# StevenWang30/R-PCC

Hardware: AMD Instinct MI355X
Metric: frames/s (64E, 64x2048 range img), projection->segmentation->model->quantise (higher is better)
Workload: dtype f32

## Files before the change

r-pcc_amd/csrc/fps_kernels.h:

```cpp
#pragma once

#define FPS_TAB_ROWS 12
#define FPS_TILE 256
#define FPS_TROWS 8

struct FpsTiling {
    int N;
    int W, H;
    int tcols;
    int T;
};
static inline FpsTiling fps_tiling_range(int H, int W) {
    FpsTiling g;
    g.N = H * W; g.W = W; g.H = H; g.tcols = (W + 31) / 32; g.T = ((H + FPS_TROWS - 1) / FPS_TROWS) * g.tcols;
    return g;
}
static inline FpsTiling fps_tiling_list(int N) {
    FpsTiling g;
    g.N = N; g.W = 0; g.H = 0; g.tcols = 0; g.T = (N + FPS_TILE - 1) / FPS_TILE;
    return g;
}

struct FpsLds {
    float4 *lo4;
// ... 115 lines not shown
    for (int e = 0; e < 4; e++) { bx[e] = cand[e] ? x[e] : qnan; by[e] = cand[e] ? y[e] : qnan; bz[e] = cand[e] ? z[e] : qnan; }
#pragma unroll
    for (int e = 0; e < 4; e += 2) {
        lo[0] = fmin3_raw(lo[0], bx[e], bx[e + 1]); hi[0] = fmax3_raw(hi[0], bx[e], bx[e + 1]);
        lo[1] = fmin3_raw(lo[1], by[e], by[e + 1]); hi[1] = fmax3_raw(hi[1], by[e], by[e + 1]);
        lo[2] = fmin3_raw(lo[2], bz[e], bz[e + 1]); hi[2] = fmax3_raw(hi[2], bz[e], bz[e + 1]);
    }
    dpp_box6(lo[0], lo[1], lo[2], hi[0], hi[1], hi[2]);
}

template <bool RANGE>
__device__ __forceinline__ void fps_load_point(const float *__restrict__ src, const float *__restrict__ rays, int k,
                                               float &x, float &y, float &z) {
    if (RANGE) {
        const float r = ld_f32(src, (uint32_t)k * 4u);
        x = r * ld_f32(rays, (uint32_t)k * 12u); y = r * ld_f32(rays, (uint32_t)k * 12u + 4u); z = r * ld_f32(rays, (uint32_t)k * 12u + 8u);
    } else {
        x = src[3 * (int64_t)k]; y = src[3 * (int64_t)k + 1]; z = src[3 * (int64_t)k + 2];
    }
}

struct FpsTileOut { float lo[3], hi[3], wt, wx, wy, wz; uint32_t widx; };

template <bool RANGE, bool VEC, bool EDGE = false>
__device__ __forceinline__ bool fps_tile_update(const FpsQuad &q, bool org_on, float t_org0, float c0, float c1, float c2,
                                                float *__restrict__ temp, bool with_box, FpsTileOut &o, bool &viol) {
    float x[4], y[4], z[4], nt[4];
    uint32_t key[4];
    bool cand[4], ch = false;
    fps_quad_xyz(q, RANGE, x, y, z);
    const bool lane_ok = q.nval > 0;
    constexpr bool QUAD = VEC && !EDGE;
#pragma unroll
    for (int e = 0; e < 4; e++) {
        float tp = (QUAD ? lane_ok : e < q.nval) ? q.tp[e] : -1.0f;
        if (RANGE && org_on && q.r[e] == 0.0f) {
            if (with_box) viol |= (QUAD ? lane_ok : e < q.nval) && tp != t_org0;
            tp = -1.0f;
        }
        cand[e] = tp >= 0.0f;
        const float dx = x[e] - c0, dy = y[e] - c1, dz = z[e] - c2;
        const float d = (dx * dx + dy * dy) + dz * dz;
        nt[e] = d < tp ? d : tp;
        key[e] = fps_val_key(nt[e]);
        const bool c = nt[e] != tp;
        ch |= c;
        if ((!VEC || (EDGE && q.nval != 4)) && c) st_f32(temp, (uint32_t)(q.p0 + e) * 4u, nt[e]);
        if (!c) nt[e] = q.tp[e];
    }
    if (QUAD && ch) st_at(reinterpret_cast<float4 *>(temp), (uint32_t)q.p0 * 4u, make_float4(nt[0], nt[1], nt[2], nt[3]));
    if (VEC && EDGE && ch && q.nval == 4) st_quad<true>(temp, (uint32_t)q.p0 * 4u, nt[0], nt[1], nt[2], nt[3]);
    if (!with_box && __ballot(ch) == 0ull) return false;
    if (with_box) fps_tile_box(x, y, z, cand, o.lo, o.hi);
    fps_tile_argmax(x, y, z, key, q.p0, o.wt, o.wx, o.wy, o.wz, o.widx);
    return true;
}

#define FPS_THREADS 1024

#define FPS_TT_BATCH 512
#define FPS_TT_SMALL 1024
#define FPS_GROUP 2
#define FPS_FLAG_FINALIZE_TEMP 1
#define FPS_FLAG_PROBED 2

template <bool RANGE, bool VEC, int FPS_TT>
__global__ __launch_bounds__(FPS_TT) void fps_tiled_kernel(const float *__restrict__ src, const float *__restrict__ rays,
                                                           float *__restrict__ temp, const int32_t *__restrict__ info,
                                                           FpsTiling g, int M, int flags, int32_t *__restrict__ out_idx,
                                                           float *__restrict__ out_cen,
                                                           const float *__restrict__ tiletab) {
    extern __shared__ __attribute__((aligned(16))) unsigned char fps_smem[];
    __shared__ unsigned long long red[FPS_TT / 64];
    __shared__ int redt[FPS_TT / 64];
    __shared__ int wcount, s_viol;
    const int T = g.T, N = g.N;
    FpsLds L(fps_smem, T);
    const int b = blockIdx.x, tid = threadIdx.x, lane = tid & 63, wave = tid >> 6;
    src += (int64_t)b * N * (RANGE ? 1 : 3);
    temp += (int64_t)b * N;
    out_idx += (int64_t)b * M;
    if (out_cen) out_cen += (int64_t)b * M * 3;
    if (M <= 0) return;
    if (!RANGE && (flags & FPS_FLAG_PROBED) && out_idx[0] < 0) return;

    int old = 0;
    if (RANGE) { old = info[RPCC_INFO * b + 1]; if (old >= N) old = 0; }
// ... 152 lines not shown
#pragma unroll
            for (int gi = 0; gi < GROUP; gi++) {
                const int ee = e + gi * NW;
                tt[gi] = (int)L.work[ee < n ? ee : n - 1];
                locate(tt[gi], q[gi]);
                fps_quad_load<RANGE, VEC>(src, rays, temp, q[gi]);
            }
#pragma unroll
            for (int gi = 0; gi < GROUP; gi++) if (e + gi * NW < n) compute_tile(tt[gi], q[gi], false);
        }
        __syncthreads();
        if (tid == 0) wcount = 0;
        select_next();
        if (lane == 0 && wave == (j & (NW - 1))) { out_idx[j] = old; if (out_cen) { out_cen[3 * j] = c0; out_cen[3 * j + 1] = c1; out_cen[3 * j + 2] = c2; } }
    }
    if (RANGE && org_on && (flags & FPS_FLAG_FINALIZE_TEMP)) {
        for (int p = tid; p < N; p += FPS_TT) {
            const float r = ld_f32(src, (uint32_t)p * 4u), tv = ld_f32(temp, (uint32_t)p * 4u);
            if (r == 0.0f && tv >= 0.0f && tv != t_org) st_f32(temp, (uint32_t)p * 4u, t_org);
        }
    }
}

template <bool RANGE, bool VEC, int FPS_TT, bool SOA, bool EDGE = false, int TPL = 1>
__device__ __forceinline__ void fps_regtab_body(const float *__restrict__ src, const float *__restrict__ rays,
                                                float *__restrict__ temp, const int32_t *__restrict__ info,
                                                FpsTiling g, int M, int flags, int32_t *__restrict__ out_idx,
                                                float *__restrict__ out_cen, const float *__restrict__ tiletab,
                                                const float *__restrict__ rays_soa, const int b) {
    constexpr int NW = FPS_TT / 64;
    TRACE_FPS_DECLS();
    TRACE_FPS_WG(0);
    __shared__ uint2 slot_k[2][NW];
    __shared__ float4 slot_c[2][NW];
    __shared__ int s_viol;
    const int T = g.T, N = g.N;
    const int tid = threadIdx.x, lane = tid & 63, wave = tid >> 6;
    src += (int64_t)b * N * (RANGE ? 1 : 3);
    temp += (int64_t)b * N;
    out_idx += (int64_t)b * M;
    if (out_cen) out_cen += (int64_t)b * M * 3;
    if (M <= 0) return;
    if (!RANGE && (flags & FPS_FLAG_PROBED) && out_idx[0] < 0) return;

    int old = 0;
    if (RANGE) { old = info[RPCC_INFO * b + 1]; if (old >= N) old = 0; }
    float c0, c1, c2;
    fps_load_point<RANGE>(src, rays, old, c0, c1, c2);
    if (tid == 0) {
        out_idx[0] = old;
        if (out_cen) { out_cen[0] = c0; out_cen[1] = c1; out_cen[2] = c2; }
        s_viol = 0;
    }
    int org_idx = N;
    if (RANGE) { org_idx = info[RPCC_INFO * b + 4]; if (org_idx < 0 || org_idx > N) org_idx = N; }
    bool org_on = RANGE && org_idx < N;
    float t_org = -1.0f;
// ... 77 lines not shown
            TRACE_FPS_VISIT(0);
#pragma unroll
            for (int u = 0; u < FPS_VISIT; u++) {
                on[u] = m != 0ull;
                l[u] = on[u] ? (int)__ffsll((long long)m) - 1 : l[0];
                sl[u] = on[u] ? cur : sl[0];
                m &= m - 1ull;
                if (TPL > 1) next();
                if (u < FPS_VISIT_UNCOND || on[u]) {
                    locate(l[u], sl[u], q[u]);
                    fps_quad_load<RANGE, VEC, SOA, EDGE>(src, SOA ? rays_soa : rays, temp, q[u], N);
                }
            }
            TRACE_FPS_VISIT(1);
#pragma unroll
            for (int u = 0; u < FPS_VISIT; u++) {
                FpsTileOut o;
                if (on[u] && fps_tile_update<RANGE, VEC, EDGE>(q[u], org_on, t_org0, c0, c1, c2, temp, with_box, o, viol)) store_entry(l[u], sl[u], o, with_box);
            }
            TRACE_FPS_VISIT(2);
        }
        if (with_box && __ballot(viol) != 0ull && lane == 0) s_viol = 1;
    };
    auto update_origin = [&]() {
        if (org_on) {
            const float d = (c0 * c0 + c1 * c1) + c2 * c2;
            t_org = d < t_org ? d : t_org;
        }
    };
    int par = 0;
    auto select_next = [&]() {
        uint32_t key = have[0] ? fps_val_key(tmax[0]) : 0u, targ_b = targ[0];
        float cx_b = cx[0], cy_b = cy[0], cz_b = cz[0];
#pragma unroll
        for (int t = 1; t < TPL; t++) {
            const uint32_t k1 = have[t] ? fps_val_key(tmax[t]) : 0u;
            const bool sec = k1 > key || (k1 == key && targ[t] < targ_b);
            key = sec ? k1 : key; targ_b = sec ? targ[t] : targ_b;
            cx_b = sec ? cx[t] : cx_b; cy_b = sec ? cy[t] : cy_b; cz_b = sec ? cz[t] : cz_b;
        }
        uint32_t vmax = dpp_max_u32(key);
        unsigned long long mm = __ballot(key == vmax);
        uint32_t imin;
        if (__popcll(mm) == 1) {
            imin = (uint32_t)__builtin_amdgcn_readlane((int)targ_b, (int)__ffsll((long long)mm) - 1);
        } else {
            imin = dpp_min_u32(key == vmax ? targ_b : 0xFFFFFFFFu);
            mm = __ballot(key == vmax && targ_b == imin);
        }
        {
            const int wl = mm ? (int)__ffsll((long long)mm) - 1 : 0;
            const float wx = u2f((uint32_t)__builtin_amdgcn_readlane((int)f2u(cx_b), wl));
            const float wy = u2f((uint32_t)__builtin_amdgcn_readlane((int)f2u(cy_b), wl));
            const float wz = u2f((uint32_t)__builtin_amdgcn_readlane((int)f2u(cz_b), wl));
            if (lane == 0) { slot_k[par][wave] = make_uint2(vmax, vmax >= FPS_KEY_MIN ? imin : 0xFFFFFFFFu); slot_c[par][wave] = make_float4(wx, wy, wz, 0.0f); }
        }
        TRACE_FPS_PHASE(3);
        __syncthreads();
        TRACE_FPS_PHASE(4);
        const uint2 kv = slot_k[par][lane % NW];
        const float4 cc = slot_c[par][lane % NW];
        par ^= 1;
        vmax = NW == 8 ? dpp_max8_u32(kv.x) : dpp_max_u32(kv.x);
        mm = __ballot(kv.x == vmax) & ((1ull << NW) - 1ull);
        if (__popcll(mm) == 1) {
            imin = (uint32_t)__builtin_amdgcn_readlane((int)kv.y, (int)__ffsll((long long)mm) - 1);
        } else {
            imin = dpp_min_u32(kv.x == vmax ? kv.y : 0xFFFFFFFFu);
            mm = __ballot(kv.x == vmax && kv.y == imin);
        }
        const int wl = mm ? (int)__ffsll((long long)mm) - 1 : 0;
        const uint32_t okey = org_on ? fps_val_key(t_org) : 0u;
        if (okey >= FPS_KEY_MIN && (okey > vmax || (okey == vmax && (uint32_t)org_idx < imin))) {
            old = org_idx;
            fps_load_point<RANGE>(src, rays, org_idx, c0, c1, c2);
        } else if (vmax < FPS_KEY_MIN || imin == 0xFFFFFFFFu) {
            old = 0;
            fps_load_point<RANGE>(src, rays, 0, c0, c1, c2);
        } else {
            old = (int)imin;
            c0 = u2f((uint32_t)__builtin_amdgcn_readlane((int)f2u(cc.x), wl));
            c1 = u2f((uint32_t)__builtin_amdgcn_readlane((int)f2u(cc.y), wl));
            c2 = u2f((uint32_t)__builtin_amdgcn_readlane((int)f2u(cc.z), wl));
        }
    };

    const bool have_tab = RANGE && tiletab != nullptr && info[RPCC_INFO * b + 3] == 1;
    if (M > 1 && have_tab) {
#pragma unroll
        for (int s = 0; s < TPL; s++) {
            if (have[s]) {
                const float4 *t4 = reinterpret_cast<const float4 *>(tiletab + (int64_t)b * FPS_TAB_ROWS * T);
                const float4 a = t4[my_t[s]], h = t4[T + my_t[s]], c = t4[2 * T + my_t[s]];
                lo0[s] = a.x; lo1[s] = a.y; lo2[s] = a.z; tmax[s] = a.w; hi0[s] = h.x; hi1[s] = h.y; hi2[s] = h.z; targ[s] = f2u(h.w);
                cx[s] = c.x; cy[s] = c.y; cz[s] = c.z;
            }
        }
        update_origin();
    } else if (M > 1) {
        __syncthreads();
        visit(have_m, true);
        __syncthreads();
        if (org_on && s_viol) {
            org_on = false; t_org = -1.0f;
            visit(have_m, true);
        }
        update_origin();
    }
    if (M > 1) {
        select_next();
        if (tid == 0) { out_idx[1] = old; if (out_cen) { out_cen[3] = c0; out_cen[4] = c1; out_cen[5] = c2; } }
    }
    TRACE_FPS_PHASE(0);
    for (int j = 2; j < M; j++) {
        unsigned long long vm[TPL];
#pragma unroll
        for (int s = 0; s < TPL; s++) {
            const float g0 = fmaxf(fmaxf(lo0[s] - c0, c0 - hi0[s]), 0.0f);
            const float g1 = fmaxf(fmaxf(lo1[s] - c1, c1 - hi1[s]), 0.0f);
            const float g2 = fmaxf(fmaxf(lo2[s] - c2, c2 - hi2[s]), 0.0f);
            const float bound = (g0 * g0 + g1 * g1) + g2 * g2;
            vm[s] = __ballot(have[s] && bound < tmax[s]);
        }
        TRACE_FPS_TILES(vm[0], j);
        TRACE_FPS_PHASE(1);
        visit(vm, false);
        TRACE_FPS_PHASE(2);
        update_origin();
        select_next();
        if (lane == 0 && wave == (j & (NW - 1))) { out_idx[j] = old; if (out_cen) { out_cen[3 * j] = c0; out_cen[3 * j + 1] = c1; out_cen[3 * j + 2] = c2; } }
        TRACE_FPS_PHASE(5);
    }
    TRACE_FPS_WG(1);
    if (RANGE && org_on && (flags & FPS_FLAG_FINALIZE_TEMP)) {
        __syncthreads();
        for (int p = tid; p < N; p += FPS_TT) {
            const float r = ld_f32(src, (uint32_t)p * 4u), tv = ld_f32(temp, (uint32_t)p * 4u);
            if (r == 0.0f && tv >= 0.0f && tv != t_org) st_f32(temp, (uint32_t)p * 4u, t_org);
        }
    }
}

template <bool RANGE, bool VEC, int FPS_TT, bool EDGE = false>
__global__ __launch_bounds__(FPS_TT) __attribute__((amdgpu_waves_per_eu(4, 8))) void fps_regtab_kernel(
    const float *__restrict__ src, const float *__restrict__ rays, float *__restrict__ temp, const int32_t *__restrict__ info, FpsTiling g, int M,
    int flags, int32_t *__restrict__ out_idx, float *__restrict__ out_cen, const float *__restrict__ tiletab) {
    fps_regtab_body<RANGE, VEC, FPS_TT, false, EDGE>(src, rays, temp, info, g, M, flags, out_idx, out_cen, tiletab, nullptr, blockIdx.x);
}
template <int FPS_TT, bool EDGE = false>
__global__ __launch_bounds__(FPS_TT) __attribute__((amdgpu_waves_per_eu(5, 8))) void fps_regtab_planar_kernel(
    const float *__restrict__ src, const float *__restrict__ rays, float *__restrict__ temp, const int32_t *__restrict__ info, FpsTiling g, int M,
    int flags, int32_t *__restrict__ out_idx, float *__restrict__ out_cen, const float *__restrict__ tiletab, const float *__restrict__ rays_soa) {
    fps_regtab_body<true, true, FPS_TT, true, EDGE>(src, rays, temp, info, g, M, flags, out_idx, out_cen, tiletab, rays_soa, blockIdx.x);
}
template <int FPS_TT, bool EDGE = false>
__global__ __launch_bounds__(FPS_TT) __attribute__((amdgpu_waves_per_eu(4, 8))) void fps_regtab_planar2_kernel(
    const float *__restrict__ src, const float *__restrict__ rays, float *__restrict__ temp, const int32_t *__restrict__ info, FpsTiling g, int M,
    int flags, int32_t *__restrict__ out_idx, float *__restrict__ out_cen, const float *__restrict__ tiletab, const float *__restrict__ rays_soa) {
    fps_regtab_body<true, true, FPS_TT, true, EDGE, 2>(src, rays, temp, info, g, M, flags, out_idx, out_cen, tiletab, rays_soa, blockIdx.x);
}
struct FpsGroupArgs {
    const float *src, *rays;
    float *temp;
    const int32_t *info;
    FpsTiling g;
    int32_t *out_idx;
    float *out_cen;
    const float *tiletab, *rays_soa;
};
struct FpsMulti {
    int n, first[RPCC_MAX_GROUPS + 1];
    int edge[RPCC_MAX_GROUPS];
    FpsGroupArgs a[RPCC_MAX_GROUPS];
};
template <int FPS_TT>
__global__ __launch_bounds__(FPS_TT) __attribute__((amdgpu_waves_per_eu(5, 8))) void fps_regtab_planar_multi_kernel(const FpsMulti m, int M, int flags) {
    const int gi = multi_group_of(m.first, m.n, blockIdx.x);
    const FpsGroupArgs &a = m.a[gi];
    const int b = (int)blockIdx.x - m.first[gi];
    if (m.edge[gi]) fps_regtab_body<true, true, FPS_TT, true, true>(a.src, a.rays, a.temp, a.info, a.g, M, flags, a.out_idx, a.out_cen, a.tiletab, a.rays_soa, b);
    else            fps_regtab_body<true, true, FPS_TT, true, false>(a.src, a.rays, a.temp, a.info, a.g, M, flags, a.out_idx, a.out_cen, a.tiletab, a.rays_soa, b);
}

#define TAB_TPW 2
#define MASK_WAVES 4
#define MASK_VGPR_ATTR
template <bool RAW, bool VEC, bool EDGE = false>
__global__ __launch_bounds__(64 * MASK_WAVES) MASK_VGPR_ATTR void ground_mask_tab_kernel(float *__restrict__ ri, const float *__restrict__ tm,
                                                              const double *__restrict__ ground, double thr, FpsTiling g,
                                                              float *__restrict__ temp, int32_t *__restrict__ info,
                                                              float *__restrict__ tiletab) {
    __shared__ int s_cnt[MASK_WAVES], s_nz[MASK_WAVES], s_first[MASK_WAVES], s_forg[MASK_WAVES];
    const int b = blockIdx.y, lane = threadIdx.x & 63, wave = threadIdx.x >> 6;
    const int P = g.N, T = g.T;
    float *ri_b = ri + (int64_t)b * P, *temp_b = temp + (int64_t)b * P;
    float4 *tab4 = reinterpret_cast<float4 *>(tiletab + (int64_t)b * FPS_TAB_ROWS * T);
    int cnt = 0, nzc = 0, first = P, forg = P;
    const int t0 = (blockIdx.x * MASK_WAVES + wave) * TAB_TPW;
    const int lrow = lane >> 3, lcol = 4 * (lane & 7);
    const float pr = ri_b[min(lane, P - 1)];
    const f32x3 pray = ld_at(reinterpret_cast<const f32x3 *>(tm), (uint32_t)min(lane, P - 1) * 12u);
    FpsQuad q[TAB_TPW];
#pragma unroll
    for (int k = 0; k < TAB_TPW; k++) {
// ... 134 lines not shown
```

r-pcc_amd/csrc/rpcc_hip.hip:

```cpp
#include <hip/hip_runtime.h>
#include <limits.h>
#include <math.h>
#include <stdint.h>
#include <stdio.h>
#include <string.h>

#include <algorithm>
#include <mutex>
#include <new>
#include <type_traits>
#include <utility>
#include <vector>
#include "../../include/rpcc_hip.h"
#include "rpcc_device.h"

using namespace rpcc;

static thread_local char g_err[512] = "";
static int set_err(int code, const char *fmt, const char *a = "", const char *b = "") {
    snprintf(g_err, sizeof(g_err), fmt, a, b);
    return code;
}
#define HIP_TRY(expr)                                                                      \
    do {                                                                                   \
        hipError_t e_ = (expr);                                                            \
        if (e_ != hipSuccess) return set_err(RPCC_ERR_HIP, "%s: %s", #expr, hipGetErrorString(e_)); \
    } while (0)
// ... 1942 lines not shown
static FpsPick fps_pick_range(int H, int W, int frames, int flags, bool quads16, bool planar) {
    const FpsTiling g = fps_tiling_range(H, W);
    if (flags & RPCC_FPS_MODE_BITS) return {FPS_MODES, FPS_THREADS, false};
    if ((flags & RPCC_FPS_BRUTEFORCE) || !fps_prunable(g)) return {FPS_ONE_PASS, FPS_THREADS, false};
    return fps_pick_pruned(g, frames, quads16, planar);
}

template <bool RANGE, int TT, bool VEC>
static int launch_fps_family(FpsFamily family, const FpsGroupArgs &a, int B, int M, int kflags, hipStream_t st) {
    if constexpr (RANGE) {
        if (family == FPS_PLANAR) fps_regtab_planar_kernel<TT, !VEC><<<B, TT, 0, st>>>(a.src, a.rays, a.temp, a.info, a.g, M, kflags, a.out_idx, a.out_cen, a.tiletab, a.rays_soa);
        if (family == FPS_PLANAR2) fps_regtab_planar2_kernel<TT, !VEC><<<B, TT, 0, st>>>(a.src, a.rays, a.temp, a.info, a.g, M, kflags, a.out_idx, a.out_cen, a.tiletab, a.rays_soa);
    }
    if (family == FPS_REG_TABLE)
        fps_regtab_kernel<RANGE, RANGE || VEC, TT, RANGE && !VEC><<<B, TT, 0, st>>>(a.src, a.rays, a.temp, a.info, a.g, M, kflags, a.out_idx, a.out_cen, a.tiletab);
    if (family == FPS_LDS_TABLE) {
        const size_t sh = fps_tiled_lds_bytes(a.g.T);
        HIP_TRY(ensure_dyn_lds(reinterpret_cast<const void *>(&fps_tiled_kernel<RANGE, VEC, TT>), (int)sh));
        fps_tiled_kernel<RANGE, VEC, TT><<<B, TT, sh, st>>>(a.src, a.rays, a.temp, a.info, a.g, M, kflags, a.out_idx, a.out_cen, a.tiletab);
    }
    LAUNCH_CHECK();
    return RPCC_OK;
}
template <bool RANGE>
static int launch_fps_tiled(const FpsPick &k, const FpsGroupArgs &a, int B, int M, int kflags, hipStream_t st) {
    if (k.threads == FPS_TT_SMALL)
        return k.unaligned ? launch_fps_family<RANGE, FPS_TT_SMALL, false>(k.family, a, B, M, kflags, st) : launch_fps_family<RANGE, FPS_TT_SMALL, true>(k.family, a, B, M, kflags, st);
    return k.unaligned ? launch_fps_family<RANGE, FPS_TT_BATCH, false>(k.family, a, B, M, kflags, st) : launch_fps_family<RANGE, FPS_TT_BATCH, true>(k.family, a, B, M, kflags, st);
}

static int fps_xyz_impl(int B, int N, int M, const float *points, float *temp, int32_t *idx, bool brute, hipStream_t st, int flags = 0) {
    ARG_TRY(B > 0 && B <= RPCC_MAX_BATCH && N > 0 && M >= 0 && points && temp && idx);
    ARG_TRY(!((flags & RPCC_FPS_FMA1) && (flags & RPCC_FPS_FMA2)));
    if (M == 0) return RPCC_OK;
    if (flags & RPCC_FPS_MODE_BITS) {
        fps_modes_kernel<false><<<B, FPS_THREADS, 0, st>>>(points, nullptr, temp, nullptr, N, M, fps_fma_of(flags),
                                                           (flags & RPCC_FPS_TIE_CUDA) ? 1 : 0, fps_pow2_down_mask(), idx, nullptr);
        LAUNCH_CHECK();
        return RPCC_OK;
    }
    const FpsTiling g = fps_tiling_list(N);
    const bool vec = (N % 4 == 0) && aligned16(points) && aligned16(temp);
    int probed = 0;
    if (!brute && fps_prunable(g)) {
        fps_list_probe_kernel<<<B, 256, 0, st>>>(points, N, M, g.T, idx);
        LAUNCH_CHECK();
        const int rc = launch_fps_tiled<false>(fps_pick_pruned(g, B, vec, false), {points, nullptr, temp, nullptr, g, idx, nullptr, nullptr, nullptr}, B, M, FPS_FLAG_PROBED, st);
        if (rc != RPCC_OK) return rc;
// ... 1289 lines not shown
    }
    if (m.n == 0) return RPCC_OK;
    return launch_ground_ransac_multi(m, st);
}
static int mixed_fps(const BatchPlan *pl, int G, hipStream_t st) {
    int rc, total = 0, tt = FPS_TT_SMALL;
    for (int i = 0; i < G; i++)
        if (pl[i].tiled && pl[i].io->timer == nullptr) total += pl[i].Bs;
    bool common[RPCC_MAX_GROUPS];
    FpsMulti m;
    m.n = 0; m.first[0] = 0;
    for (int i = 0; i < G; i++) {
        const BatchPlan &p = pl[i];
        const FpsPick k = fps_pick_range(p.g.H, p.g.W, total, p.io->flags, range_quads16(p.g.W, p.io->ri, p.temp, p.io->tm), true);
        common[i] = k.family == FPS_PLANAR && p.io->timer == nullptr;
        if (!common[i]) continue;
        tt = k.threads;
        m.a[m.n] = {p.io->ri, p.io->tm, p.temp, p.io->info, fps_tiling_range(p.g.H, p.g.W), p.io->cen_pix, p.io->centers, p.tiletab, p.rays_soa};
        m.edge[m.n] = k.unaligned ? 1 : 0;
        m.first[m.n + 1] = m.first[m.n] + p.Bs;
        m.n++;
    }
    if (m.n > 0) {
        if (tt == FPS_TT_SMALL) fps_regtab_planar_multi_kernel<FPS_TT_SMALL><<<m.first[m.n], FPS_TT_SMALL, 0, st>>>(m, pl[0].M, 0);
        else                    fps_regtab_planar_multi_kernel<FPS_TT_BATCH><<<m.first[m.n], FPS_TT_BATCH, 0, st>>>(m, pl[0].M, 0);
        LAUNCH_CHECK();
    }
    for (int i = 0; i < G; i++)
        if (!common[i] && (rc = run_stage<uint8_t>(pl[i], ST_FPS, st))) return rc;
    return RPCC_OK;
}
static int mixed_planes(const BatchPlan *pl, int G, hipStream_t st) {
    PlaneMulti m;
    m.n = 0; m.first[0] = 0;
    const int M = pl[0].M, K = M + 2, wpg = PL_THREADS / 64, groups = (K + wpg - 1) / wpg;
    for (int i = 0; i < G; i++) {
        const BatchPlan &p = pl[i];
        if (p.io->model_method == 0) continue;
        m.a[m.n] = plane_group_args(p.io->tm, p.io->ground, p.Bs, p.P, M, p.io->plane_cos_cut, (uint32_t)p.io->plane_seed, p.io->frame_ids,
                                    p.io->model, p.io->counts, p.ws, p.extra, nullptr);
        m.first[m.n + 1] = m.first[m.n] + p.Bs * (K - 2) + p.Bs * groups;
        m.n++;
    }
    if (m.n == 0) return RPCC_OK;
    plane_model_multi_kernel<10><<<m.first[m.n], PL_THREADS, 0, st>>>(m, M, kpad(M), PL_BIG);
    LAUNCH_CHECK();
    return RPCC_OK;
}
// ... 233 lines not shown
```

Measured before the change: 358,500.

## Speculatively process two FPS centres per round with guessed next centre

Adds a speculative 'pair' mode to the tiled FPS kernel. Each round updates distances for the current centre and also for a guessed next centre, which is the runner-up candidate still valid after the current update. The second centre's tile updates are staged in LDS and committed only if the guess proves correct, so one barrier and reduction round can yield two centres. It also emits v_subrev with a scalar operand for the distance subtraction. The cost is extra LDS staging, more register pressure, pause/backoff logic when staging overflows, and correctness risk, which a new simulator script is meant to check.

```diff
diff --git a/r-pcc_amd/csrc/fps_kernels.h b/r-pcc_amd/csrc/fps_kernels.h
--- a/r-pcc_amd/csrc/fps_kernels.h
+++ b/r-pcc_amd/csrc/fps_kernels.h
@@ -161,6 +161,24 @@
 
 struct FpsTileOut { float lo[3], hi[3], wt, wx, wy, wz; uint32_t widx; };
 
+__device__ __forceinline__ float fps_point_min(float x, float y, float z, float c0, float c1, float c2, float tp) {
+    const float dx = x - c0, dy = y - c1, dz = z - c2;
+    const float d = (dx * dx + dy * dy) + dz * dz;
+    return d < tp ? d : tp;
+}
+__device__ __forceinline__ float fps_sub_uniform(float x, float c) {
+    float r;
+    asm("v_subrev_f32_e32 %0, %1, %2" : "=v"(r) : "s"(c), "v"(x));
+    return r;
+}
+template <bool UNI>
+__device__ __forceinline__ float fps_point_min_t(float x, float y, float z, float c0, float c1, float c2, float tp) {
+    if (!UNI) return fps_point_min(x, y, z, c0, c1, c2, tp);
+    const float dx = fps_sub_uniform(x, c0), dy = fps_sub_uniform(y, c1), dz = fps_sub_uniform(z, c2);
+    const float d = (dx * dx + dy * dy) + dz * dz;
+    return d < tp ? d : tp;
+}
+
 template <bool RANGE, bool VEC, bool EDGE = false>
 __device__ __forceinline__ bool fps_tile_update(const FpsQuad &q, bool org_on, float t_org0, float c0, float c1, float c2,
                                                 float *__restrict__ temp, bool with_box, FpsTileOut &o, bool &viol) {
@@ -178,9 +196,7 @@
             tp = -1.0f;
         }
         cand[e] = tp >= 0.0f;
-        const float dx = x[e] - c0, dy = y[e] - c1, dz = z[e] - c2;
-        const float d = (dx * dx + dy * dy) + dz * dz;
-        nt[e] = d < tp ? d : tp;
+        nt[e] = fps_point_min(x[e], y[e], z[e], c0, c1, c2, tp);
         key[e] = fps_val_key(nt[e]);
         const bool c = nt[e] != tp;
         ch |= c;
@@ -195,13 +211,87 @@
     return true;
 }
 
+template <bool RANGE, bool VEC, bool EDGE = false>
+__device__ __forceinline__ void fps_pair_begin(const FpsQuad &q, bool org_on, bool in_b, float4 *__restrict__ stage, float (&x)[4], float (&y)[4],
+                                               float (&z)[4], float (&tp)[4]) {
+    fps_quad_xyz(q, RANGE, x, y, z);
+    const bool lane_ok = q.nval > 0;
+    constexpr bool QUAD = VEC && !EDGE;
+    if (in_b) *stage = make_float4(q.tp[0], q.tp[1], q.tp[2], q.tp[3]);
+#pragma unroll
+    for (int e = 0; e < 4; e++) {
+        tp[e] = (QUAD ? lane_ok : e < q.nval) ? q.tp[e] : -1.0f;
+        if (RANGE && org_on && q.r[e] == 0.0f) tp[e] = -1.0f;
+    }
+}
+template <bool VEC, bool EDGE = false>
+__device__ __forceinline__ bool fps_pair_centre(const FpsQuad &q, const float (&x)[4], const float (&y)[4], const float (&z)[4], float (&tp)[4],
+                                                float c0, float c1, float c2, float *__restrict__ temp, FpsTileOut &o) {
+    constexpr bool QUAD = VEC && !EDGE;
+    bool ch = false;
+    float wb[4];
+    uint32_t key[4];
+#pragma unroll
+    for (int e = 0; e < 4; e++) {
+        const float nt = fps_point_min_t<true>(x[e], y[e], z[e], c0, c1, c2, tp[e]);
+        const bool c = nt != tp[e];
+        ch |= c;
+        if ((!VEC || (EDGE && q.nval != 4)) && c) st_f32(temp, (uint32_t)(q.p0 + e) * 4u, nt);
+        wb[e] = c ? nt : q.tp[e];
+        tp[e] = nt;
+    }
+    if (QUAD && ch) st_at(reinterpret_cast<float4 *>(temp), (uint32_t)q.p0 * 4u, make_float4(wb[0], wb[1], wb[2], wb[3]));
+    if (VEC && EDGE && ch && q.nval == 4) st_quad<true>(temp, (uint32_t)q.p0 * 4u, wb[0], wb[1], wb[2], wb[3]);
+    if (__ballot(ch) == 0ull) return false;
+#pragma unroll
+    for (int e = 0; e < 4; e++) key[e] = fps_val_key(tp[e]);
+    fps_tile_argmax(x, y, z, key, q.p0, o.wt, o.wx, o.wy, o.wz, o.widx);
+    return true;
+}
+__device__ __forceinline__ bool fps_pair_guess(const FpsQuad &q, const float (&x)[4], const float (&y)[4], const float (&z)[4], float (&tp)[4],
+                                               float g0, float g1, float g2, float4 *__restrict__ stage, FpsTileOut &o) {
+    bool chg = false;
+    uint32_t key[4];
+#pragma unroll
+    for (int e = 0; e < 4; e++) {
+        const float nt = fps_point_min_t<true>(x[e], y[e], z[e], g0, g1, g2, tp[e]);
+        chg |= nt != tp[e];
+        tp[e] = nt;
+    }
+    if (__ballot(chg) == 0ull) return false;
+#pragma unroll
+    for (int e = 0; e < 4; e++) key[e] = fps_val_key(tp[e]);
+    fps_tile_argmax(x, y, z, key, q.p0, o.wt, o.wx, o.wy, o.wz, o.widx);
+    const float4 raw = *stage;
+    *stage = make_float4(tp[0] >= 0.0f ? tp[0] : raw.x, tp[1] >= 0.0f ? tp[1] : raw.y, tp[2] >= 0.0f ? tp[2] : raw.z, tp[3] >= 0.0f ? tp[3] : raw.w);
+    return true;
+}
+template <bool VEC, bool EDGE>
+__device__ __forceinline__ void fps_quad_flush(const FpsQuad &q, float *__restrict__ temp, const float4 v) {
+    if (VEC && !EDGE) { if (q.nval > 0) st_at(reinterpret_cast<float4 *>(temp), (uint32_t)q.p0 * 4u, v); return; }
+    if (VEC && EDGE && q.nval == 4) { st_quad<true>(temp, (uint32_t)q.p0 * 4u, v.x, v.y, v.z, v.w); return; }
+    const float a[4] = {v.x, v.y, v.z, v.w};
+#pragma unroll
+    for (int e = 0; e < 4; e++) if (e < q.nval) st_f32(temp, (uint32_t)(q.p0 + e) * 4u, a[e]);
+}
+
 #define FPS_THREADS 1024
 
 #define FPS_TT_BATCH 512
 #define FPS_TT_SMALL 1024
 #define FPS_GROUP 2
 #define FPS_FLAG_FINALIZE_TEMP 1
+#define FPS_FLAG_PAIRS 4
 #define FPS_FLAG_PROBED 2
+
+#define FPS_PAIR_CAP 2
+#define FPS_PAIR_PAUSE_MAX 2
+template <int NW>
+struct FpsPairLds {
+    float4 quad[NW][FPS_PAIR_CAP][64];
+    float4 ent[NW][FPS_PAIR_CAP];
+    uint2 enti[NW][FPS_PAIR_CAP];
+};
 
 template <bool RANGE, bool VEC, int FPS_TT>
 __global__ __launch_bounds__(FPS_TT) void fps_tiled_kernel(const float *__restrict__ src, const float *__restrict__ rays,
@@ -400,17 +490,20 @@
     }
 }
 
-template <bool RANGE, bool VEC, int FPS_TT, bool SOA, bool EDGE = false, int TPL = 1>
+template <bool RANGE, bool VEC, int FPS_TT, bool SOA, bool EDGE = false, int TPL = 1, bool PAIRS = true>
 __device__ __forceinline__ void fps_regtab_body(const float *__restrict__ src, const float *__restrict__ rays,
                                                 float *__restrict__ temp, const int32_t *__restrict__ info,
                                                 FpsTiling g, int M, int flags, int32_t *__restrict__ out_idx,
                                                 float *__restrict__ out_cen, const float *__restrict__ tiletab,
-                                                const float *__restrict__ rays_soa, const int b) {
+                                                const float *__restrict__ rays_soa, const int b,
+                                                FpsPairLds<FPS_TT / 64> &PL) {
     constexpr int NW = FPS_TT / 64;
     TRACE_FPS_DECLS();
     TRACE_FPS_WG(0);
     __shared__ uint2 slot_k[2][NW];
     __shared__ float4 slot_c[2][NW];
+    __shared__ uint2 slot_k2[2][NW];
+    __shared__ float4 slot_c2[2][NW];
     __shared__ int s_viol;
     const int T = g.T, N = g.N;
     const int tid = threadIdx.x, lane = tid & 63, wave = tid >> 6;
@@ -534,6 +627,55 @@
         }
         if (with_box && __ballot(viol) != 0ull && lane == 0) s_viol = 1;
     };
+    bool have_g = false;
+    uint32_t gi = 0u;
+    float g0 = 0.0f, g1 = 0.0f, g2 = 0.0f;
+    auto visit_pair = [&](const unsigned long long (&va)[TPL], const unsigned long long (&vb)[TPL], int &ns) {
+        unsigned long long mu[TPL];
+#pragma unroll
+        for (int t = 0; t < TPL; t++) mu[t] = va[t] | vb[t];
+        unsigned long long m = mu[0];
+        int cur = 0;
+        auto next = [&]() {
+#pragma unroll
+            for (int t = 1; t < TPL; t++) if (m == 0ull && cur < t) { m = mu[t]; cur = t; }
+        };
+        if (TPL > 1) next();
+        while (m) {
+            int l[FPS_VISIT], sl[FPS_VISIT];
+            bool on[FPS_VISIT];
+            FpsQuad q[FPS_VISIT];
+#pragma unroll
+            for (int u = 0; u < FPS_VISIT; u++) {
+                on[u] = m != 0ull;
+                l[u] = on[u] ? (int)__ffsll((long long)m) - 1 : l[0];
+                sl[u] = on[u] ? cur : sl[0];
+                m &= m - 1ull;
+                if (TPL > 1) next();
+                if (u < FPS_VISIT_UNCOND || on[u]) {
+                    locate(l[u], sl[u], q[u]);
+                    fps_quad_load<RANGE, VEC, SOA, EDGE>(src, SOA ? rays_soa : rays, temp, q[u], N);
+                }
+            }
+#pragma unroll
+            for (int u = 0; u < FPS_VISIT; u++) {
+                if (!on[u]) continue;
+                unsigned long long a = va[0], bm = vb[0];
+#pragma unroll
+                for (int t = 1; t < TPL; t++) if (sl[u] == t) { a = va[t]; bm = vb[t]; }
+                const bool in_a = (a >> l[u]) & 1ull, in_b = (bm >> l[u]) & 1ull;
+                float4 *stage = &PL.quad[wave][min(ns, FPS_PAIR_CAP - 1)][lane];
+                float x[4], y[4], z[4], tp[4];
+                FpsTileOut o;
+                fps_pair_begin<RANGE, VEC, EDGE>(q[u], org_on, in_b, stage, x, y, z, tp);
+                if (in_a && fps_pair_centre<VEC, EDGE>(q[u], x, y, z, tp, c0, c1, c2, temp, o)) store_entry(l[u], sl[u], o, false);
+                if (in_b && fps_pair_guess(q[u], x, y, z, tp, g0, g1, g2, stage, o)) {
+                    if (lane == 0) { PL.ent[wave][ns] = make_float4(o.wx, o.wy, o.wz, o.wt); PL.enti[wave][ns] = make_uint2(o.widx, (uint32_t)(l[u] | (sl[u] << 8))); }
+                    ns++;
+                }
+            }
+        }
+    };
     auto update_origin = [&]() {
         if (org_on) {
             const float d = (c0 * c0 + c1 * c1) + c2 * c2;
@@ -541,60 +683,95 @@
         }
     };
     int par = 0;
-    auto select_next = [&]() {
-        uint32_t key = have[0] ? fps_val_key(tmax[0]) : 0u, targ_b = targ[0];
-        float cx_b = cx[0], cy_b = cy[0], cz_b = cz[0];
-#pragma unroll
-        for (int t = 1; t < TPL; t++) {
-            const uint32_t k1 = have[t] ? fps_val_key(tmax[t]) : 0u;
-            const bool sec = k1 > key || (k1 == key && targ[t] < targ_b);
-            key = sec ? k1 : key; targ_b = sec ? targ[t] : targ_b;
-            cx_b = sec ? cx[t] : cx_b; cy_b = sec ? cy[t] : cy_b; cz_b = sec ? cz[t] : cz_b;
-        }
-        uint32_t vmax = dpp_max_u32(key);
+    auto wave_best = [&](int ns, uint32_t &vmax, uint32_t &imin, float &wx, float &wy, float &wz) {
+        uint32_t key = 0u, targ_b = 0u;
+        float cx_b = 0.0f, cy_b = 0.0f, cz_b = 0.0f;
+#pragma unroll
+        for (int t = 0; t < TPL; t++) {
+            uint32_t k1 = have[t] ? fps_val_key(tmax[t]) : 0u, a1 = targ[t];
+            float x1 = cx[t], y1 = cy[t], z1 = cz[t];
+            for (int i = 0; i < ns; i++) {
+                const float4 e = PL.ent[wave][i];
+                const uint2 ei = PL.enti[wave][i];
+                if ((int)ei.y == (lane | (t << 8))) { k1 = fps_val_key(e.w); a1 = ei.x; x1 = e.x; y1 = e.y; z1 = e.z; }
+            }
+            const bool sec = t > 0 && (k1 > key || (k1 == key && a1 < targ_b));
+            key = (t == 0 || sec) ? k1 : key; targ_b = (t == 0 || sec) ? a1 : targ_b;
+            cx_b = (t == 0 || sec) ? x1 : cx_b; cy_b = (t == 0 || sec) ? y1 : cy_b; cz_b = (t == 0 || sec) ? z1 : cz_b;
+        }
+        vmax = dpp_max_u32(key);
         unsigned long long mm = __ballot(key == vmax);
-        uint32_t imin;
         if (__popcll(mm) == 1) {
             imin = (uint32_t)__builtin_amdgcn_readlane((int)targ_b, (int)__ffsll((long long)mm) - 1);
         } else {
             imin = dpp_min_u32(key == vmax ? targ_b : 0xFFFFFFFFu);
             mm = __ballot(key == vmax && targ_b == imin);
         }
-        {
-            const int wl = mm ? (int)__ffsll((long long)mm) - 1 : 0;
-            const float wx = u2f((uint32_t)__builtin_amdgcn_readlane((int)f2u(cx_b), wl));
-            const float wy = u2f((uint32_t)__builtin_amdgcn_readlane((int)f2u(cy_b), wl));
-            const float wz = u2f((uint32_t)__builtin_amdgcn_readlane((int)f2u(cz_b), wl));
-            if (lane == 0) { slot_k[par][wave] = make_uint2(vmax, vmax >= FPS_KEY_MIN ? imin : 0xFFFFFFFFu); slot_c[par][wave] = make_float4(wx, wy, wz, 0.0f); }
-        }
+        const int wl = mm ? (int)__ffsll((long long)mm) - 1 : 0;
+        wx = u2f((uint32_t)__builtin_amdgcn_readlane((int)f2u(cx_b), wl));
+        wy = u2f((uint32_t)__builtin_amdgcn_readlane((int)f2u(cy_b), wl));
+        wz = u2f((uint32_t)__builtin_amdgcn_readlane((int)f2u(cz_b), wl));
+        if (vmax < FPS_KEY_MIN) imin = 0xFFFFFFFFu;
+    };
+    auto pick = [&](const uint2 kv, const float4 cc) -> bool {
+        const uint32_t vmax = NW == 8 ? dpp_max8_u32(kv.x) : dpp_max_u32(kv.x);
+        unsigned long long mm = __ballot(kv.x == vmax) & ((1ull << NW) - 1ull);
+        uint32_t imin;
+        if (__popcll(mm) == 1) {
+            imin = (uint32_t)__builtin_amdgcn_readlane((int)kv.y, (int)__ffsll((long long)mm) - 1);
+        } else {
+            imin = dpp_min_u32(kv.x == vmax ? kv.y : 0xFFFFFFFFu);
+            mm = __ballot(kv.x == vmax && kv.y == imin);
+        }
+        const int wl = mm ? (int)__ffsll((long long)mm) - 1 : 0;
+        const uint32_t okey = org_on ? fps_val_key(t_org) : 0u;
+        if (okey >= FPS_KEY_MIN && (okey > vmax || (okey == vmax && (uint32_t)org_idx < imin))) {
+            old = org_idx;
+            fps_load_point<RANGE>(src, rays, org_idx, c0, c1, c2);
+            return false;
+        } else if (vmax < FPS_KEY_MIN || imin == 0xFFFFFFFFu) {
+            old = 0;
+            fps_load_point<RANGE>(src, rays, 0, c0, c1, c2);
+            return false;
+        }
+        old = (int)imin;
+        c0 = u2f((uint32_t)__builtin_amdgcn_readlane((int)f2u(cc.x), wl));
+        c1 = u2f((uint32_t)__builtin_amdgcn_readlane((int)f2u(cc.y), wl));
+        c2 = u2f((uint32_t)__builtin_amdgcn_readlane((int)f2u(cc.z), wl));
+        return true;
+    };
+    const bool pairs_on = PAIRS && (flags & FPS_FLAG_PAIRS) != 0;
+    auto make_guess = [&](const uint2 kv, const float4 cc) {
+        const float val = fps_key_val(kv.x);
+        const bool ok = kv.x >= FPS_KEY_MIN && kv.y != (uint32_t)old && !(fps_point_min(cc.x, cc.y, cc.z, c0, c1, c2, val) != val);
+        const uint32_t gk = ok ? kv.x : 0u;
+        const uint32_t gmax = NW == 8 ? dpp_max8_u32(gk) : dpp_max_u32(gk);
+        have_g = gmax >= FPS_KEY_MIN;
+        unsigned long long mm = __ballot(gk == gmax) & ((1ull << NW) - 1ull);
+        if (__popcll(mm) == 1) {
+            gi = (uint32_t)__builtin_amdgcn_readlane((int)kv.y, (int)__ffsll((long long)mm) - 1);
+        } else {
+            gi = dpp_min_u32(gk == gmax ? kv.y : 0xFFFFFFFFu);
+            mm = __ballot(gk == gmax && kv.y == gi);
+        }
+        const int wl = mm ? (int)__ffsll((long long)mm) - 1 : 0;
+        g0 = u2f((uint32_t)__builtin_amdgcn_readlane((int)f2u(cc.x), wl));
+        g1 = u2f((uint32_t)__builtin_amdgcn_readlane((int)f2u(cc.y), wl));
+        g2 = u2f((uint32_t)__builtin_amdgcn_readlane((int)f2u(cc.z), wl));
+    };
+    auto select_next = [&]() {
+        uint32_t vmax, imin;
+        float wx, wy, wz;
+        wave_best(0, vmax, imin, wx, wy, wz);
+        if (lane == 0) { slot_k[par][wave] = make_uint2(vmax, imin); slot_c[par][wave] = make_float4(wx, wy, wz, 0.0f); }
         TRACE_FPS_PHASE(3);
         __syncthreads();
         TRACE_FPS_PHASE(4);
         const uint2 kv = slot_k[par][lane % NW];
         const float4 cc = slot_c[par][lane % NW];
         par ^= 1;
-        vmax = NW == 8 ? dpp_max8_u32(kv.x) : dpp_max_u32(kv.x);
-        mm = __ballot(kv.x == vmax) & ((1ull << NW) - 1ull);
-        if (__popcll(mm) == 1) {
-            imin = (uint32_t)__builtin_amdgcn_readlane((int)kv.y, (int)__ffsll((long long)mm) - 1);
-        } else {
-            imin = dpp_min_u32(kv.x == vmax ? kv.y : 0xFFFFFFFFu);
-            mm = __ballot(kv.x == vmax && kv.y == imin);
-        }
-        const int wl = mm ? (int)__ffsll((long long)mm) - 1 : 0;
-        const uint32_t okey = org_on ? fps_val_key(t_org) : 0u;
-        if (okey >= FPS_KEY_MIN && (okey > vmax || (okey == vmax && (uint32_t)org_idx < imin))) {
-            old = org_idx;
-            fps_load_point<RANGE>(src, rays, org_idx, c0, c1, c2);
-        } else if (vmax < FPS_KEY_MIN || imin == 0xFFFFFFFFu) {
-            old = 0;
-            fps_load_point<RANGE>(src, rays, 0, c0, c1, c2);
-        } else {
-            old = (int)imin;
-            c0 = u2f((uint32_t)__builtin_amdgcn_readlane((int)f2u(cc.x), wl));
-            c1 = u2f((uint32_t)__builtin_amdgcn_readlane((int)f2u(cc.y), wl));
-            c2 = u2f((uint32_t)__builtin_amdgcn_readlane((int)f2u(cc.z), wl));
-        }
+        pick(kv, cc);
+        if (pairs_on) make_guess(kv, cc);
     };
 
     const bool have_tab = RANGE && tiletab != nullptr && info[RPCC_INFO * b + 3] == 1;
@@ -624,24 +801,88 @@
         if (tid == 0) { out_idx[1] = old; if (out_cen) { out_cen[3] = c0; out_cen[4] = c1; out_cen[5] = c2; } }
     }
     TRACE_FPS_PHASE(0);
-    for (int j = 2; j < M; j++) {
-        unsigned long long vm[TPL];
+    auto write_centre = [&](int j) {
+        if (lane == 0 && wave == (j & (NW - 1))) { out_idx[j] = old; if (out_cen) { out_cen[3 * j] = c0; out_cen[3 * j + 1] = c1; out_cen[3 * j + 2] = c2; } }
+    };
+    int pause = 0, pause_len = 1;
+    for (int j = 2; j < M;) {
+        const bool attempt = pairs_on && have_g && j <= M - 2 && pause == 0;
+        pause = pause > 0 ? pause - 1 : 0;
+        unsigned long long va[TPL], vb[TPL];
+        int nb = 0;
 #pragma unroll
         for (int s = 0; s < TPL; s++) {
-            const float g0 = fmaxf(fmaxf(lo0[s] - c0, c0 - hi0[s]), 0.0f);
-            const float g1 = fmaxf(fmaxf(lo1[s] - c1, c1 - hi1[s]), 0.0f);
-            const float g2 = fmaxf(fmaxf(lo2[s] - c2, c2 - hi2[s]), 0.0f);
-            const float bound = (g0 * g0 + g1 * g1) + g2 * g2;
-            vm[s] = __ballot(have[s] && bound < tmax[s]);
-        }
-        TRACE_FPS_TILES(vm[0], j);
+            const float b0 = fmaxf(fmaxf(lo0[s] - c0, c0 - hi0[s]), 0.0f);
+            const float b1 = fmaxf(fmaxf(lo1[s] - c1, c1 - hi1[s]), 0.0f);
+            const float b2 = fmaxf(fmaxf(lo2[s] - c2, c2 - hi2[s]), 0.0f);
+            const float bound = (b0 * b0 + b1 * b1) + b2 * b2;
+            va[s] = __ballot(have[s] && bound < tmax[s]);
+            vb[s] = 0ull;
+            if (attempt) {
+                const float e0 = fmaxf(fmaxf(lo0[s] - g0, g0 - hi0[s]), 0.0f);
+                const float e1 = fmaxf(fmaxf(lo1[s] - g1, g1 - hi1[s]), 0.0f);
+                const float e2 = fmaxf(fmaxf(lo2[s] - g2, g2 - hi2[s]), 0.0f);
+                const float bound_g = (e0 * e0 + e1 * e1) + e2 * e2;
+                vb[s] = __ballot(have[s] && bound_g < tmax[s]);
+                nb += __popcll(vb[s]);
+            }
+        }
+        TRACE_FPS_TILES(va[0], j);
         TRACE_FPS_PHASE(1);
-        visit(vm, false);
+        const bool decline = nb > FPS_PAIR_CAP;
+        if (decline) {
+#pragma unroll
+            for (int s = 0; s < TPL; s++) vb[s] = 0ull;
+        }
+        int ns = 0;
+        visit_pair(va, vb, ns);
         TRACE_FPS_PHASE(2);
         update_origin();
-        select_next();
-        if (lane == 0 && wave == (j & (NW - 1))) { out_idx[j] = old; if (out_cen) { out_cen[3 * j] = c0; out_cen[3 * j + 1] = c1; out_cen[3 * j + 2] = c2; } }
-        TRACE_FPS_PHASE(5);
+        {
+            uint32_t vmax, imin;
+            float wx, wy, wz;
+            wave_best(0, vmax, imin, wx, wy, wz);
+            if (lane == 0) { slot_k[par][wave] = make_uint2(vmax, imin); slot_c[par][wave] = make_float4(wx, wy, wz, decline ? 1.0f : 0.0f); }
+            if (attempt) {
+                if (ns > 0) wave_best(ns, vmax, imin, wx, wy, wz);
+                if (lane == 0) { slot_k2[par][wave] = make_uint2(vmax, imin); slot_c2[par][wave] = make_float4(wx, wy, wz, 0.0f); }
+            }
+        }
+        TRACE_FPS_PHASE(3);
+        __syncthreads();
+        TRACE_FPS_PHASE(4);
+        const uint2 kv = slot_k[par][lane % NW];
+        const float4 cc = slot_c[par][lane % NW];
+        const int par2 = par;
+        par ^= 1;
+        const bool declined = __ballot(cc.w != 0.0f) != 0ull;
+        const bool from_tile = pick(kv, cc);
+        write_centre(j);
+        j++;
+        if (attempt && from_tile && (uint32_t)old == gi && !declined) {
+            const uint2 kv2 = slot_k2[par2][lane % NW];
+            const float4 cc2 = slot_c2[par2][lane % NW];
+            update_origin();
+            for (int i = 0; i < ns; i++) {
+                const float4 e = PL.ent[wave][i];
+                const uint2 ei = PL.enti[wave][i];
+                const int l = __builtin_amdgcn_readfirstlane((int)(ei.y & 0xFFu)), sl = __builtin_amdgcn_readfirstlane((int)(ei.y >> 8));
+                FpsQuad q;
+                locate(l, sl, q);
+                fps_quad_flush<VEC, EDGE>(q, temp, PL.quad[wave][i][lane]);
+                FpsTileOut o;
+                o.wt = e.w; o.wx = e.x; o.wy = e.y; o.wz = e.z; o.widx = ei.x;
+                store_entry(l, sl, o, false);
+            }
+            pick(kv2, cc2);
+            write_centre(j);
+            j++;
+            make_guess(kv2, cc2);
+            pause_len = 1;
+        } else {
+            if (pairs_on) make_guess(kv, cc);
+            if (attempt && declined) { pause = pause_len; pause_len = min(2 * pause_len, FPS_PAIR_PAUSE_MAX); }
+        }
     }
     TRACE_FPS_WG(1);
     if (RANGE && org_on && (flags & FPS_FLAG_FINALIZE_TEMP)) {
@@ -657,19 +898,22 @@
 __global__ __launch_bounds__(FPS_TT) __attribute__((amdgpu_waves_per_eu(4, 8))) void fps_regtab_kernel(
     const float *__restrict__ src, const float *__restrict__ rays, float *__restrict__ temp, const int32_t *__restrict__ info, FpsTiling g, int M,
     int flags, int32_t *__restrict__ out_idx, float *__restrict__ out_cen, const float *__restrict__ tiletab) {
-    fps_regtab_body<RANGE, VEC, FPS_TT, false, EDGE>(src, rays, temp, info, g, M, flags, out_idx, out_cen, tiletab, nullptr, blockIdx.x);
+    __shared__ FpsPairLds<FPS_TT / 64> pair_lds;
+    fps_regtab_body<RANGE, VEC, FPS_TT, false, EDGE>(src, rays, temp, info, g, M, flags, out_idx, out_cen, tiletab, nullptr, blockIdx.x, pair_lds);
 }
 template <int FPS_TT, bool EDGE = false>
 __global__ __launch_bounds__(FPS_TT) __attribute__((amdgpu_waves_per_eu(5, 8))) void fps_regtab_planar_kernel(
     const float *__restrict__ src, const float *__restrict__ rays, float *__restrict__ temp, const int32_t *__restrict__ info, FpsTiling g, int M,
     int flags, int32_t *__restrict__ out_idx, float *__restrict__ out_cen, const float *__restrict__ tiletab, const float *__restrict__ rays_soa) {
-    fps_regtab_body<true, true, FPS_TT, true, EDGE>(src, rays, temp, info, g, M, flags, out_idx, out_cen, tiletab, rays_soa, blockIdx.x);
+    __shared__ FpsPairLds<FPS_TT / 64> pair_lds;
+    fps_regtab_body<true, true, FPS_TT, true, EDGE, 1, !EDGE>(src, rays, temp, info, g, M, flags, out_idx, out_cen, tiletab, rays_soa, blockIdx.x, pair_lds);
 }
 template <int FPS_TT, bool EDGE = false>
 __global__ __launch_bounds__(FPS_TT) __attribute__((amdgpu_waves_per_eu(4, 8))) void fps_regtab_planar2_kernel(
     const float *__restrict__ src, const float *__restrict__ rays, float *__restrict__ temp, const int32_t *__restrict__ info, FpsTiling g, int M,
     int flags, int32_t *__restrict__ out_idx, float *__restrict__ out_cen, const float *__restrict__ tiletab, const float *__restrict__ rays_soa) {
-    fps_regtab_body<true, true, FPS_TT, true, EDGE, 2>(src, rays, temp, info, g, M, flags, out_idx, out_cen, tiletab, rays_soa, blockIdx.x);
+    __shared__ FpsPairLds<FPS_TT / 64> pair_lds;
+    fps_regtab_body<true, true, FPS_TT, true, EDGE, 2>(src, rays, temp, info, g, M, flags, out_idx, out_cen, tiletab, rays_soa, blockIdx.x, pair_lds);
 }
 struct FpsGroupArgs {
     const float *src, *rays;
@@ -687,11 +931,12 @@
 };
 template <int FPS_TT>
 __global__ __launch_bounds__(FPS_TT) __attribute__((amdgpu_waves_per_eu(5, 8))) void fps_regtab_planar_multi_kernel(const FpsMulti m, int M, int flags) {
+    __shared__ FpsPairLds<FPS_TT / 64> pair_lds;
     const int gi = multi_group_of(m.first, m.n, blockIdx.x);
     const FpsGroupArgs &a = m.a[gi];
     const int b = (int)blockIdx.x - m.first[gi];
-    if (m.edge[gi]) fps_regtab_body<true, true, FPS_TT, true, true>(a.src, a.rays, a.temp, a.info, a.g, M, flags, a.out_idx, a.out_cen, a.tiletab, a.rays_soa, b);
-    else            fps_regtab_body<true, true, FPS_TT, true, false>(a.src, a.rays, a.temp, a.info, a.g, M, flags, a.out_idx, a.out_cen, a.tiletab, a.rays_soa, b);
+    if (m.edge[gi]) fps_regtab_body<true, true, FPS_TT, true, true, 1, false>(a.src, a.rays, a.temp, a.info, a.g, M, flags, a.out_idx, a.out_cen, a.tiletab, a.rays_soa, b, pair_lds);
+    else            fps_regtab_body<true, true, FPS_TT, true, false>(a.src, a.rays, a.temp, a.info, a.g, M, flags, a.out_idx, a.out_cen, a.tiletab, a.rays_soa, b, pair_lds);
 }
 
 #define TAB_TPW 2
diff --git a/r-pcc_amd/csrc/rpcc_hip.hip b/r-pcc_amd/csrc/rpcc_hip.hip
--- a/r-pcc_amd/csrc/rpcc_hip.hip
+++ b/r-pcc_amd/csrc/rpcc_hip.hip
@@ -3,6 +3,7 @@
 #include <math.h>
 #include <stdint.h>
 #include <stdio.h>
+#include <stdlib.h>
 #include <string.h>
 
 #include <algorithm>
@@ -1991,8 +1992,13 @@
     LAUNCH_CHECK();
     return RPCC_OK;
 }
+static int fps_pairs_flag() {
+    static const int f = [] { const char *e = getenv("RPCC_FPS_PAIRS"); return (e && e[0] == '0' && e[1] == 0) ? 0 : FPS_FLAG_PAIRS; }();
+    return f;
+}
 template <bool RANGE>
 static int launch_fps_tiled(const FpsPick &k, const FpsGroupArgs &a, int B, int M, int kflags, hipStream_t st) {
+    kflags |= fps_pairs_flag();
     if (k.threads == FPS_TT_SMALL)
         return k.unaligned ? launch_fps_family<RANGE, FPS_TT_SMALL, false>(k.family, a, B, M, kflags, st) : launch_fps_family<RANGE, FPS_TT_SMALL, true>(k.family, a, B, M, kflags, st);
     return k.unaligned ? launch_fps_family<RANGE, FPS_TT_BATCH, false>(k.family, a, B, M, kflags, st) : launch_fps_family<RANGE, FPS_TT_BATCH, true>(k.family, a, B, M, kflags, st);
@@ -3328,8 +3334,8 @@
         m.n++;
     }
     if (m.n > 0) {
-        if (tt == FPS_TT_SMALL) fps_regtab_planar_multi_kernel<FPS_TT_SMALL><<<m.first[m.n], FPS_TT_SMALL, 0, st>>>(m, pl[0].M, 0);
-        else                    fps_regtab_planar_multi_kernel<FPS_TT_BATCH><<<m.first[m.n], FPS_TT_BATCH, 0, st>>>(m, pl[0].M, 0);
+        if (tt == FPS_TT_SMALL) fps_regtab_planar_multi_kernel<FPS_TT_SMALL><<<m.first[m.n], FPS_TT_SMALL, 0, st>>>(m, pl[0].M, fps_pairs_flag());
+        else                    fps_regtab_planar_multi_kernel<FPS_TT_BATCH><<<m.first[m.n], FPS_TT_BATCH, 0, st>>>(m, pl[0].M, fps_pairs_flag());
         LAUNCH_CHECK();
     }
     for (int i = 0; i < G; i++)
diff --git a/tools_dev/sim_fps_pairs.py b/tools_dev/sim_fps_pairs.py
--- /dev/null
+++ b/tools_dev/sim_fps_pairs.py
@@ -0,0 +1,225 @@
+import argparse
+import os
+import sys
+
+import numpy as np
+
+sys.path.insert(0, os.path.dirname(os.path.dirname(os.path.abspath(__file__))))
+import rpcc_amd
+from rpcc_amd import synth
+from oracle import oracle as orc
+
+TR, TC = 8, 32
+GROUND = np.array([0.002, -0.004, -0.99999, -1.73])
+F = np.float32
+
+
+def _dist(p, c):
+    d = (p - c).astype(F)
+    return ((d[..., 0] * d[..., 0]).astype(F) + (d[..., 1] * d[..., 1]).astype(F)).astype(F) + (d[..., 2] * d[..., 2]).astype(F)
+
+
+def frame_inputs(fid, H, W, scene="default", ground=GROUND):
+    g = orc.LidarGeom(H=H, W=W)
+    tm = orc.transform_map(g)
+    xyz = synth.make_frame(fid, H, W, scene=scene).numpy()
+    ri = orc.project(xyz, g)
+    return ri.reshape(H, W), tm, np.asarray(ground, np.float64)
+
+
+def simulate(ri, tm, ground, M, nw=8, cap=2, pause_max=2, pairs=True, threshold=0.1):
+    H, W = ri.shape
+    P = H * W
+    pc = orc.backproject(ri, tm).reshape(-1, 3).astype(F)
+    mask = (orc.vertical_residual(pc.reshape(H, W, 3), ground) > threshold).reshape(-1)
+    riv = ri.reshape(-1)
+    tcols = (W + TC - 1) // TC
+    T = ((H + TR - 1) // TR) * tcols
+    pix = np.arange(P)
+    tile = ((pix // W) // TR) * tcols + (pix % W) // TC
+    tr_, tc_ = np.arange(T) // tcols, np.arange(T) % tcols
+    wave_of = (tr_ * tcols + (tc_ + 3 * tr_) % tcols) % nw
+    org = mask & (riv == 0)
+    org_on = bool(org.any())
+    org_idx = int(np.flatnonzero(org)[0]) if org_on else P
+    cand = mask & ~org
+    members = [np.flatnonzero(cand & (tile == t)) for t in range(T)]
+    lo = np.full((T, 3), np.inf, F)
+    hi = np.full((T, 3), -np.inf, F)
+    for t in range(T):
+        if members[t].size:
+            lo[t], hi[t] = pc[members[t]].min(0), pc[members[t]].max(0)
+    temp = np.where(mask, F(1e10), F(-1))
+    tmax = np.full(T, -1, F)
+    targ = np.zeros(T, np.int64)
+
+    def entry(t, vals):
+        m = members[t]
+        if not m.size:
+            return F(-1), 0
+        k = int(np.argmax(vals))
+        return vals[k], int(m[k])
+
+    def bound(c):
+        gap = np.maximum(np.maximum(lo - c, c - hi), F(0)).astype(F)
+        return ((gap[:, 0] * gap[:, 0]).astype(F) + (gap[:, 1] * gap[:, 1]).astype(F)).astype(F) + (gap[:, 2] * gap[:, 2]).astype(F)
+
+    first = int(np.flatnonzero(mask)[0])
+    c = pc[first].copy()
+    idx = [first]
+    t_org = F(1e10) if org_on else F(-1)
+
+    def upd_org(t_org, c):
+        if not org_on:
+            return t_org
+        d = ((c[0] * c[0]).astype(F) + (c[1] * c[1]).astype(F)).astype(F) + (c[2] * c[2]).astype(F)
+        return d if d < t_org else t_org
+
+    for t in range(T):
+        m = members[t]
+        if m.size:
+            temp[m] = np.minimum(temp[m], _dist(pc[m], c))
+        tmax[t], targ[t] = entry(t, temp[m])
+    t_org = upd_org(t_org, c)
+
+    def candidates(tmx, tag):
+        out = []
+        for w in range(nw):
+            ts = np.flatnonzero(wave_of == w)
+            v = tmx[ts]
+            if not ts.size or v.max() < 0:
+                out.append((F(-1), -1))
+                continue
+            best = ts[v == v.max()]
+            out.append((v.max(), int(tag[best].min())))
+        return out
+
+    def pick(cands, t_org):
+        vals = np.array([v for v, _ in cands], F)
+        vmax = vals.max()
+        imin = min((i for v, i in cands if v == vmax), default=-1) if vmax >= 0 else -1
+        if org_on and t_org >= 0 and (t_org > vmax or (t_org == vmax and org_idx < imin)):
+            return org_idx, False
+        if vmax < 0:
+            return 0, False
+        return imin, True
+
+    def guess(cands, old):
+        best = None
+        for v, i in cands:
+            if v < 0 or i == old:
+                continue
+            if _dist(pc[i], pc[old]) < v:
+                continue
+            if best is None or v > best[0] or (v == best[0] and i < best[1]):
+                best = (v, i)
+        return None if best is None else best[1]
+
+    st = dict(rounds=0, commits=0, wrong=0, declines=0, over_cap=0, both=0, last_rule=0, attempts=0)
+    if M > 1:
+        cands = candidates(tmax, targ)
+        old, _ = pick(cands, t_org)
+        idx.append(old)
+        g = guess(cands, old) if pairs else None
+    j, pause, pause_len = 2, 0, 1
+    while j < M:
+        st["rounds"] += 1
+        c = pc[old]
+        if pairs and g is not None and pause == 0 and j == M - 1:
+            st["last_rule"] += 1
+        attempt = pairs and g is not None and j <= M - 2 and pause == 0
+        pause = max(pause - 1, 0)
+        A = bound(c) < tmax
+        stage = {}
+        declined = False
+        if attempt:
+            st["attempts"] += 1
+            Bm = bound(pc[g]) < tmax
+            for w in range(nw):
+                ts = np.flatnonzero(Bm & (wave_of == w))
+                if ts.size > cap:
+                    declined = True
+                    st["over_cap"] += 1
+                    Bm[ts] = False
+        for t in np.flatnonzero(A):
+            m = members[t]
+            temp[m] = np.minimum(temp[m], _dist(pc[m], c))
+            tmax[t], targ[t] = entry(t, temp[m])
+        t_org = upd_org(t_org, c)
+        tmax2, targ2 = tmax, targ
+        if attempt:
+            tmax2, targ2 = tmax.copy(), targ.copy()
+            for t in np.flatnonzero(Bm):
+                m = members[t]
+                v2 = np.minimum(temp[m], _dist(pc[m], pc[g]))
+                if (v2 != temp[m]).any():
+                    stage[t] = v2
+                    tmax2[t], targ2[t] = entry(t, v2)
+                    st["both"] += bool(A[t])
+        cands = candidates(tmax, targ)
+        old, from_tile = pick(cands, t_org)
+        idx.append(old)
+        j += 1
+        if attempt and from_tile and old == g and not declined:
+            st["commits"] += 1
+            t_org = upd_org(t_org, pc[old])
+            for t, v2 in stage.items():
+                temp[members[t]] = v2
+            tmax, targ = tmax2, targ2
+            cands = candidates(tmax, targ)
+            old, _ = pick(cands, t_org)
+            idx.append(old)
+            j += 1
+            g = guess(cands, old)
+            pause_len = 1
+        else:
+            if attempt and declined:
+                st["declines"] += 1
+                pause, pause_len = pause_len, min(2 * pause_len, pause_max)
+            elif attempt:
+                st["wrong"] += 1
+            g = guess(cands, old) if pairs else None
+    if org_on:
+        temp[org] = t_org
+    st["idx"] = np.array(idx[:M], np.int64)
+    st["temp"] = temp
+    return st
+
+
+def reference(ri, tm, ground, M, threshold=0.1):
+    H, W = ri.shape
+    pc = orc.backproject(ri, tm).reshape(-1, 3).astype(F)
+    mask = (orc.vertical_residual(pc.reshape(H, W, 3), ground) > threshold).reshape(-1)
+    where = np.flatnonzero(mask)
+    pixidx = where[orc.fps(pc[where], M)]
+    temp = np.where(mask, F(1e10), F(-1))
+    for k in pixidx[:max(M - 1, 1)]:
+        temp[where] = np.minimum(temp[where], _dist(pc[where], pc[k]))
+    return pixidx, temp
+
+
+def run_checked(ri, tm, ground, M, **kw):
+    st = simulate(ri, tm, ground, M, **kw)
+    pixidx, temp = reference(ri, tm, ground, M)
+    assert np.array_equal(st["idx"], pixidx), "the pair rounds changed the centre sequence"
+    assert np.array_equal(st["temp"].view(np.uint32), temp.view(np.uint32)), "final temp is not the minimum over the first M - 1 centres"
+    return st
+
+
+if __name__ == "__main__":
+    ap = argparse.ArgumentParser()
+    ap.add_argument("--H", type=int, default=64)
+    ap.add_argument("--W", type=int, default=2048)
+    ap.add_argument("--M", type=int, default=100)
+    ap.add_argument("--nw", type=int, default=8)
+    ap.add_argument("--cap", type=int, default=2)
+    ap.add_argument("--pause-max", type=int, default=2)
+    ap.add_argument("--scene", default="default")
+    ap.add_argument("frames", nargs="*", type=int, default=[0, 5])
+    a = ap.parse_args()
+    for fid in a.frames:
+        ri, tm, gm = frame_inputs(fid, a.H, a.W, a.scene)
+        st = run_checked(ri, tm, gm, a.M, nw=a.nw, cap=a.cap, pause_max=a.pause_max)
+        print("%s frame %d: %d rounds for %d centres; commits %d, wrong guesses %d, declined rounds %d (wavefronts over the cap %d), "
+              "tiles hit by both %d, attempts %d, last-centre rule %d" % (a.scene, fid, st["rounds"], a.M - 1, st["commits"], st["wrong"], st["declines"],
+                                                                           st["over_cap"], st["both"], st["attempts"], st["last_rule"]))
```

Measured after the change: 348,000. 0.971x the previous value.
